# codgodtao/TMDiff

Hardware: AMD Instinct MI355X
Metric: UNet denoise-steps/sec (8-ch 64x64, batch 32) (higher is better)
Workload: dtype f32; 1 GPU; BASELINE configs[1]: batch-32 8-ch 64x64 tiles, DDPM p_sample steps of the T=1000 cosine schedule, channel_multiplier [32,64,128,256], full UNet forward (both branches) + fused DDPM update per step; batch_per_gpu=32, parallelism=batch-parallel x1, weights=key-hashed random init, text_embedding=fixed synthetic 768-d

## Files before the change

include/tmdiff_hip.h:

```cpp
#ifndef TMDIFF_HIP_H
#define TMDIFF_HIP_H

#include <stddef.h>
#include <stdint.h>

#ifdef __cplusplus
extern "C" {
#endif

#define TMDIFF_ABI_VERSION 6

#define TMDIFF_OK 0
#define TMDIFF_E_INVALID (-1)
#define TMDIFF_E_UNSUPPORTED (-2)
#define TMDIFF_E_LAUNCH (-3)

typedef void* tmdiff_stream_t;

int tmdiff_version(void);
const char* tmdiff_last_error_string(void);

typedef struct tmdiff_conv3d_desc {
  int32_t B, N, H, W;
  int32_t Cin, Cout;
// ... 140 lines not shown
int tmdiff_conv3d_prologue_bwd_add(const tmdiff_conv3d_desc* d, const float* gp, float* const dx_seg[3],
                                   const float* const add_seg[3], float* d_shift, float* d_scale, void* workspace,
                                   tmdiff_stream_t stream);

int tmdiff_stem_fwd(const float* xin, const float* pan, const float* ms, const float* w, const float* bias, float* y,
                    int32_t B, int32_t Cout, int32_t N, int32_t H, int32_t W, int32_t apply_silu,
                    tmdiff_stream_t stream);
int tmdiff_stem_fwd_scaled(const float* xin, const float* pan, const float* ms, const float* w, const float* bias,
                           const float* out_scale, int32_t out_scale_stride, float* y, int32_t B, int32_t Cout, int32_t N,
                           int32_t H, int32_t W, int32_t apply_silu, tmdiff_stream_t stream);
int tmdiff_stem_fwd_pack_bf16(const float* xin, const float* pan, const float* ms, const float* w, const float* bias,
                              const float* out_scale, int32_t out_scale_stride, void* units, int32_t B, int32_t Cout, int32_t N,
                              int32_t H, int32_t W, int32_t apply_silu, tmdiff_stream_t stream);
int tmdiff_head_fwd(const float* x, const float* w, const float* scale, int32_t scale_stride, float* y, int32_t B,
                    int32_t C, int64_t P, tmdiff_stream_t stream);
int tmdiff_stem_bwd(const float* xin, const float* pan, const float* ms, const float* w, const float* bias,
                    const float* gy, float* dwb, int32_t B, int32_t Cout, int32_t N, int32_t H, int32_t W,
                    tmdiff_stream_t stream);
int tmdiff_stem_bwd_input(const float* xin, const float* pan, const float* ms, const float* w, const float* bias,
                          const float* gy, float* dx, float* dpan, int32_t B, int32_t Cout, int32_t N, int32_t H,
                          int32_t W, tmdiff_stream_t stream);
int tmdiff_head_bwd(const float* x, const float* w, const float* scale, const float* gy, float* dx, float* dws,
                    int32_t B, int32_t C, int64_t P, tmdiff_stream_t stream);

typedef struct tmdiff_plane_prologue {
  const float* shift;
  const float* scale;
  int32_t shift_stride, scale_stride;
  int32_t C, n_per_channel;
  int32_t act;
} tmdiff_plane_prologue;
int tmdiff_haar_dwt2d_pro(const float* x, float* ll, float* lh, float* hl, float* hh, int64_t planes, int32_t H, int32_t W,
                          float ll_scale, float hi_scale, const tmdiff_plane_prologue* ll_prologue, tmdiff_stream_t stream);
int tmdiff_haar_idwt2d_pro(const float* const ll[2], int32_t n_ll, const float* lh, const float* hl, const float* hh,
                           int64_t hi_planes_per_batch, int64_t hi_batch_stride, float* const out[2], int64_t planes,
                           int32_t h, int32_t w, float in_scale, const tmdiff_plane_prologue* out0_prologue,
                           tmdiff_stream_t stream);
int tmdiff_haar_dwt2d_pack_bf16(const float* x, void* ll_units, float* lh, float* hl, float* hh, int32_t B, int32_t C,
                                int32_t N, int32_t H, int32_t W, float ll_scale, float hi_scale,
                                const tmdiff_plane_prologue* ll_prologue, tmdiff_stream_t stream);
int tmdiff_haar_idwt2d_pack_bf16(const float* ll0, const float* ll1, const float* stacked_bands, void* out0_units, float* out1,
                                 int32_t B, int32_t C, int32_t N, int32_t h, int32_t w, float in_scale,
                                 const tmdiff_plane_prologue* out0_prologue, tmdiff_stream_t stream);
int tmdiff_haar_dwt2d(const float* x, float* ll, float* lh, float* hl, float* hh, int64_t planes, int32_t H,
                      int32_t W, float ll_scale, float hi_scale, tmdiff_stream_t stream);
int tmdiff_haar_idwt2d(const float* const ll[2], int32_t n_ll, const float* lh, const float* hl, const float* hh,
                       int64_t hi_planes_per_batch, int64_t hi_batch_stride, float* const out[2], int64_t planes,
                       int32_t h, int32_t w, float in_scale, tmdiff_stream_t stream);

int tmdiff_linear_fwd(const float* x, const float* w, const float* bias, float* y, int32_t B, int32_t I, int32_t O,
                      int32_t act, tmdiff_stream_t stream);
int tmdiff_gamma_embedding(const float* t, const float* freqs, float* emb, int32_t B, int32_t dim,
                           tmdiff_stream_t stream);
int tmdiff_linear_bwd(const float* x, const float* w, const float* bias, const float* gy, float* gu_scratch,
                      float* dx, float* dw, float* db, int32_t B, int32_t I, int32_t O, int32_t act,
                      tmdiff_stream_t stream);

int tmdiff_ddpm_step(const float* x, const float* eps, const float* noise, const float* ms, float* out,
                     float* img_out, int64_t n, float c_recip, float c_recipm1, float coef1, float coef2,
                     float sigma, int32_t clip, tmdiff_stream_t stream);
int tmdiff_axpby(const float* const in[4], const float coef[4], int32_t n_in, float* out, int64_t n,
                 tmdiff_stream_t stream);
int tmdiff_ddpm_step_dev(const float* x, const float* eps, const float* noise, const float* ms, float* out, float* frames,
                         int64_t n, const int32_t* step, const float* coef, int32_t T, int32_t frame_every, int32_t clip,
                         tmdiff_stream_t stream);
int tmdiff_sampler_tick(int32_t* step, float* time_in, int32_t B, int32_t set_to, tmdiff_stream_t stream);
int tmdiff_ddpm_frame_slot(int32_t t, int32_t T, int32_t frame_every);
typedef struct tmdiff_mt_entry {
  float* out;
  const float* a;
  const float* b;
  int64_t n;
} tmdiff_mt_entry;
int32_t tmdiff_multi_axpby_chunk(void);
int tmdiff_multi_axpby(const tmdiff_mt_entry* tensors_dev, const int32_t* chunk_tensor_dev, const int32_t* chunk_index_dev,
                       int32_t n_chunks, float ca, float cb, tmdiff_stream_t stream);
typedef struct tmdiff_adamw_entry {
  float* p;
  const float* g;
  float* m;
  float* v;
  int64_t n;
} tmdiff_adamw_entry;
int tmdiff_multi_adamw(const tmdiff_adamw_entry* tensors_dev, const int32_t* chunk_tensor_dev, const int32_t* chunk_index_dev,
                       int32_t n_chunks, const float* lr_dev, const float* step_dev, float beta1, float beta2, float eps,
                       float weight_decay, tmdiff_stream_t stream);
size_t tmdiff_multi_sqnorm_workspace_bytes(int32_t n_chunks);
int tmdiff_multi_sqnorm_partial(const tmdiff_adamw_entry* tensors_dev, const int32_t* chunk_tensor_dev,
                                const int32_t* chunk_index_dev, int32_t n_chunks, double* partials_dev, tmdiff_stream_t stream);
int tmdiff_multi_sqnorm_finish(const double* partials_dev, int32_t n_partials, float max_norm, float* norm_dev, float* coef_dev,
                               float* ok_dev, tmdiff_stream_t stream);
int tmdiff_multi_adamw_scaled(const tmdiff_adamw_entry* tensors_dev, const int32_t* chunk_tensor_dev,
                              const int32_t* chunk_index_dev, int32_t n_chunks, const float* lr_dev, const float* step_dev,
                              float beta1, float beta2, float eps, float weight_decay, const float* coef_dev, const float* ok_dev,
                              tmdiff_stream_t stream);
int tmdiff_x0_from_model(const float* x, const float* model_out, float* x0, int64_t n, float alpha, float sigma,
                         int32_t model_is_x_start, tmdiff_stream_t stream);
size_t tmdiff_abs_quantile_workspace_bytes(int32_t B, int64_t n_per_sample);
int tmdiff_abs_quantile_clamp(float* x0, int32_t B, int64_t n_per_sample, float q, float max_val, void* workspace,
                              tmdiff_stream_t stream);
int tmdiff_add(const float* a, const float* b, float* out, int64_t n, float sign_b, tmdiff_stream_t stream);
int tmdiff_q_sample(const float* x0, const float* noise, const float* a, float* out, int32_t B, int64_t n_per_sample,
                    tmdiff_stream_t stream);

int32_t tmdiff_tile_plan(int32_t L, int32_t tile, int32_t overlap, int32_t* origins, int32_t capacity);
int tmdiff_tile_supported(int32_t B, int32_t C, int32_t H, int32_t W, int32_t tile, int32_t overlap);
// ... 112 lines not shown
```

tmdiff_amd/Hyper_unet_general.py:

```python
import math

import torch
import torch.nn as nn

from . import ops, routing

PROMPTS = ("QB", "WV3", "GF2", "WV2", "WV4")

def synthetic_text_embeddings(seed=1234):
    out = {}
    for k, name in enumerate(PROMPTS):
        g = torch.Generator(device="cpu").manual_seed(seed + k)
        out[name] = torch.randn(1, 768, generator=g)
    return out


class Swish(nn.Module):

    def forward(self, x):
        raise RuntimeError("Swish is fused into the HIP kernels; it is never called as a module")



_MASK_FN = None
# ... 512 lines not shown
    @staticmethod
    def _tensor_key(t):
        return (t.data_ptr(), t._version, tuple(t.shape), tuple(t.stride()))

    def begin_condition_cache(self, PAN, MS, prompt):
        with torch.no_grad():
            self._cond = self._condition(self._prepare(), PAN, MS, prompt)
        self._cond["key"] = (self._tensor_key(PAN), self._tensor_key(MS), prompt)

    def add_condition_cache(self, PAN, MS, prompt):
        P = self._prepare()
        if self._cond is None:
            raise RuntimeError("add_condition_cache: no open condition cache (call begin_condition_cache first)")
        with torch.no_grad():
            cond = self._condition(P, PAN, MS, prompt)
        cond["key"] = (self._tensor_key(PAN), self._tensor_key(MS), prompt)
        self._cond.setdefault("more", []).append(cond)

    def end_condition_cache(self):
        self._cond = None

    def invalidate_prepared(self):
        self._prep = None
        self._cond = None
        self.__dict__.pop("_train_pack", None)
        self.__dict__.pop("_train_pack_wino", None)
        self.__dict__.pop("_train_pack_bf16", None)

    _DERIVED = ("_train_pack", "_train_pack_wino", "_train_pack_bf16", "_emb_dev", "_freqs_dev", "_side_stream")

    def __getstate__(self):
        state = {k: v for k, v in self.__dict__.items() if k not in self._DERIVED}
        state["_prep"] = state["_cond"] = None
        return state

    def forward(self, x_t, t_input, PAN=None, MS=None, prompt=None):
        if torch.is_grad_enabled() and (any(p.requires_grad for p in self.parameters()) or any(
                torch.is_tensor(t) and t.requires_grad for t in (x_t, PAN, MS))):
            return self.forward_train(x_t, t_input, PAN, MS, prompt)
        with torch.no_grad():
            return self._forward_infer(x_t, t_input, PAN, MS, prompt)

    def _forward_infer(self, x_t, t_input, PAN, MS, prompt):
        P = self._prepare()
        cond = self._cond
        key = (self._tensor_key(PAN), self._tensor_key(MS), prompt)
        if cond is not None and cond.get("key") != key:
            cond = next((c for c in cond.get("more", ()) if c["key"] == key), None)
        if cond is None:
            cond = self._condition(P, PAN, MS, prompt)
        b = x_t.shape[0]
        t = t_input.reshape(-1).to(device=x_t.device, dtype=torch.float32)
        t = (t if t.numel() == b else t.expand(b)).contiguous()
        g = ops.gamma_embedding(t, P["freqs"], self.inter_dim)
        e = ops.linear(g, self.embed[0].weight.detach(), self.embed[0].bias.detach(), act=True)
        temb = ops.linear(e, self.embed[2].weight.detach(), self.embed[2].bias.detach(), act=True)
        S = {"shift": P["shift_bank"].run(temb), "scale": cond["scale"]}

        fuse_c, fuse = self._producer_fuse(P)
        spec = lambda **k: self._spec(P, S, **k) if fuse_c else None
        h, hp = self._stem(P, S, "conv2", "down1.conv20.dense1", xin=x_t.contiguous())
        hs = [h]
        for dn, nxt in (("down1", "down2.conv20"), ("down2", "down3.conv20"), ("down3", "middle1")):
            h, ha, hq, s2d = self._resblock(P, S, dn + ".conv20", [h], flag=False, pre=hp, emit=spec(), want_ll=True, to_conv0=True)
            h, hp, _ = self._down(P, S, dn + ".down", h, flag=False, want_high=False, pre=ha,
                                  emit=spec(shift=nxt + ".dense1"), fuse=fuse, xq=hq, s2d=s2d)
            hs.append(h)
        h, _ = self._resblock(P, S, "middle1", [hs[3]], flag=False, pre=hp)
        for lvl, upn in ((3, "up1"), (2, "up2"), (1, "up3")):
            h, ha = self._resblock(P, S, upn + ".conv20", [h, cond[f"h{lvl}"], hs[lvl]], flag=False, emit=spec())
            h = self._up(P, S, upn + ".up1", h, cond[f"bands{lvl}"], pre=ha, fuse=fuse)
        h, hp = self._resblock(P, S, "final.conv20", [h, cond["h0"], hs[0]], flag=False, emit=spec(shift="final.conv21.dense1"))
        for k in (1, 2, 3):
            h, hp = self._resblock(P, S, f"final.conv2{k}", [h], flag=False, pre=hp,
                                   emit=spec(shift=f"final.conv2{k + 1}.dense1") if k < 3 else None)
        sc = self._spec(P, S, scale="final.dense2")
        return ops.head(h, self.final.conv24.weight.detach().reshape(-1), sc["scale"], sc["scale_stride"])

    def forward_train(self, x_t, t_input, PAN=None, MS=None, prompt=None):
        from . import autograd as A
        dev = x_t.device
        if dev.type != "cuda":
            raise RuntimeError("tmdiff_amd.WavBEST runs on the HIP kernels only: move the module to a GPU (.cuda())")
        b = x_t.shape[0]
        pk = self.__dict__.get("_train_pack")
        if pk is None or pk.convs[0][0].device != dev:
            self.__dict__.pop("_train_pack_bf16", None)
            pk = self.__dict__["_train_pack"] = ops.PackedWeights(
                [(m.weight, m.groups) for m in self.modules()
                 if isinstance(m, nn.Conv3d) and m.in_channels > 1 and m.out_channels > 1])
        ops.PACKED = pk.refresh()
        wk = self.__dict__.get("_train_pack_wino")
        if wk is None:
            wk = self.__dict__["_train_pack_wino"] = ops.WinoPackedWeights(owner=[w for w, _ in pk.convs])
        ops.WINO_PACKED = wk.refresh() if ops.config.wino_multipack else None
        if ops.config.grad_bf16 and "_train_pack_bf16" not in self.__dict__:
            self.__dict__["_train_pack_bf16"] = ops.Bf16DgradWeights(owner=[w for w, _ in pk.convs])
        ops.BF16_DGRAD = self.__dict__["_train_pack_bf16"] if ops.config.grad_bf16 else None
        lin = lambda seq, i, x, act: A.linear(x, seq[i].weight, seq[i].bias, act=act)
        pe = self._prompt_rows(prompt, b, dev)
        pemb = lin(self.embed2, 4, lin(self.embed2, 2, lin(self.embed2, 0, pe, True), True), True)
        t = t_input.reshape(-1).to(device=dev, dtype=torch.float32)
        t = (t if t.numel() == b else t.expand(b)).contiguous()
        fr = self.__dict__.get("_freqs_dev")
        if fr is None or fr.device != dev:
            fr = self.__dict__["_freqs_dev"] = self._freqs_cpu.to(dev)
        g = ops.gamma_embedding(t, fr, self.inter_dim)
        temb = lin(self.embed, 2, lin(self.embed, 0, g, True), True)

        shift_layers, scale_layers = self._projection_layers()
# ... 50 lines not shown
```

tmdiff_amd/_lib.py:

```python
import ctypes as C
import os

_HERE = os.path.dirname(os.path.abspath(__file__))
LIB_PATH = os.environ.get("TMDIFF_HIP_LIB") or os.path.join(_HERE, "libtmdiff_hip.so")

c_float_p = C.POINTER(C.c_float)
vp = C.c_void_p


class Conv3dDesc(C.Structure):
    _fields_ = [
        ("B", C.c_int32), ("N", C.c_int32), ("H", C.c_int32), ("W", C.c_int32),
        ("Cin", C.c_int32), ("Cout", C.c_int32),
        ("groups", C.c_int32), ("ksize", C.c_int32), ("nseg", C.c_int32),
        ("seg_c", C.c_int32 * 3),
        ("seg_x", vp * 3),
        ("w_packed", vp), ("bias", vp), ("bias_scale", C.c_float),
        ("in_shift", vp), ("in_scale", vp), ("in_shift_stride", C.c_int32), ("in_scale_stride", C.c_int32),
        ("in_mask", vp), ("in_act", C.c_int32),
        ("residual", vp), ("out_scale", C.c_float),
        ("y", vp),
        ("y2", vp), ("y2_shift", vp), ("y2_scale", vp), ("y2_shift_stride", C.c_int32), ("y2_scale_stride", C.c_int32),
        ("y2_act", C.c_int32), ("y2_bf16", C.c_int32), ("x_bf16", C.c_int32),
        ("splitk_ws", vp), ("splitk_ws_bytes", C.c_int64),
# ... 27 lines not shown
    "tmdiff_conv3d_wf_workspace_bytes": (C.c_size_t, [C.POINTER(Conv3dDesc)]),
    "tmdiff_conv3d_wf_splitk_workspace_bytes": (C.c_size_t, [C.POINTER(Conv3dDesc)]),
    "tmdiff_conv3d_wf_fwd": (C.c_int, [C.POINTER(Conv3dDesc), vp, vp]),
    "tmdiff_conv3d_wino_fwd": (C.c_int, [C.POINTER(Conv3dDesc), vp, vp]),
    "tmdiff_conv3d_wino_fwd_planes": (C.c_int, [C.POINTER(Conv3dDesc), vp, C.c_int32, vp, C.c_int32, vp]),
    "tmdiff_conv3d_wino_fwd_xp": (C.c_int, [C.POINTER(Conv3dDesc), vp, C.c_int32, vp, vp]),
    "tmdiff_conv3d_wino_fwd_stage": (C.c_int, [C.POINTER(Conv3dDesc), vp, C.c_int32, vp]),
    "tmdiff_conv3d_prologue_fwd": (C.c_int, [C.POINTER(Conv3dDesc), vp, vp]),
    "tmdiff_conv3d_ll_supported": (C.c_int, [C.POINTER(Conv3dDesc)]),
    "tmdiff_conv3d_ll_splitk_workspace_bytes": (C.c_size_t, [C.POINTER(Conv3dDesc)]),
    "tmdiff_conv3d_ll_packed_bytes": (C.c_size_t, [C.c_int32, C.c_int32]),
    "tmdiff_conv3d_ll_pack_weights": (C.c_int, [vp, vp, C.c_int32, C.c_int32, C.c_float, vp]),
    "tmdiff_conv3d_ll_fwd": (C.c_int, [C.POINTER(Conv3dDesc), C.c_float, vp]),
    "tmdiff_conv3d_packed_bf16_bytes": (C.c_size_t, [C.c_int32, C.c_int32, C.c_int32, C.c_int32]),
    "tmdiff_conv3d_pack_weights_bf16": (C.c_int, [vp, vp, C.c_int32, C.c_int32, C.c_int32, C.c_int32, vp]),
    "tmdiff_conv3d_bf16_workspace_bytes": (C.c_size_t, [C.POINTER(Conv3dDesc)]),
    "tmdiff_conv3d_fwd_bf16": (C.c_int, [C.POINTER(Conv3dDesc), vp, vp]),
    "tmdiff_conv3d_wgrad_workspace_bytes": (C.c_size_t, [C.POINTER(Conv3dDesc)]),
    "tmdiff_conv3d_wgrad": (C.c_int, [C.POINTER(Conv3dDesc), vp, vp, vp, vp]),
    "tmdiff_conv3d_wgrad_bias": (C.c_int, [C.POINTER(Conv3dDesc), vp, vp, vp, vp, vp]),
    "tmdiff_conv3d_wf_plan": (C.c_int32, [C.c_int32] * 8 + [C.POINTER(C.c_int64)]),
    "tmdiff_conv3d_wfll_supported": (C.c_int, [C.POINTER(Conv3dDesc)]),
    "tmdiff_conv3d_wfll_packed_bytes": (C.c_size_t, [C.c_int32, C.c_int32]),
    "tmdiff_conv3d_wfll_pack_weights": (C.c_int, [vp, vp, C.c_int32, C.c_int32, C.c_float, vp]),
    "tmdiff_conv3d_wfll_splitk_workspace_bytes": (C.c_size_t, [C.POINTER(Conv3dDesc)]),
    "tmdiff_conv3d_wfll_fwd": (C.c_int, [C.POINTER(Conv3dDesc), C.c_float, vp]),
    "tmdiff_conv3d_wgrad_wino_supported": (C.c_int, [C.POINTER(Conv3dDesc)]),
    "tmdiff_conv3d_wgrad_wino_workspace_bytes": (C.c_size_t, [C.POINTER(Conv3dDesc)]),
    "tmdiff_conv3d_wgrad_wino": (C.c_int, [C.POINTER(Conv3dDesc), vp, vp, vp, vp]),
    "tmdiff_conv3d_wgrad_wino_bias": (C.c_int, [C.POINTER(Conv3dDesc), vp, vp, vp, vp, vp]),
    "tmdiff_conv3d_pack_weights_bf16_dgrad": (C.c_int, [vp, vp, C.c_int32, C.c_int32, C.c_int32, C.c_int32, vp]),
    "tmdiff_conv3d_wgrad_bf16_supported": (C.c_int, [C.POINTER(Conv3dDesc)]),
    "tmdiff_conv3d_wgrad_bf16_workspace_bytes": (C.c_size_t, [C.POINTER(Conv3dDesc)]),
    "tmdiff_conv3d_wgrad_bf16_slots": (C.c_int32, [C.POINTER(Conv3dDesc)]),
    "tmdiff_conv3d_wgrad_bf16": (C.c_int, [C.POINTER(Conv3dDesc), vp, vp, vp, vp, vp]),
    "tmdiff_channel_sum": (C.c_int, [vp, vp, C.c_int32, C.c_int32, C.c_int64, C.c_float, vp]),
    "tmdiff_conv3d_prologue_bwd": (C.c_int, [C.POINTER(Conv3dDesc), vp, vp * 3, C.c_int32 * 3, vp, vp, vp]),
    "tmdiff_conv3d_prologue_bwd_workspace_bytes": (C.c_size_t, [C.POINTER(Conv3dDesc)]),
    "tmdiff_conv3d_prologue_bwd_ws": (C.c_int, [C.POINTER(Conv3dDesc), vp, vp * 3, C.c_int32 * 3, vp, vp, vp, vp]),
    "tmdiff_conv3d_prologue_bwd_add": (C.c_int, [C.POINTER(Conv3dDesc), vp, vp * 3, vp * 3, vp, vp, vp, vp]),
    "tmdiff_stem_bwd": (C.c_int, [vp, vp, vp, vp, vp, vp, vp, C.c_int32, C.c_int32, C.c_int32, C.c_int32, C.c_int32, vp]),
    "tmdiff_stem_bwd_input": (C.c_int, [vp, vp, vp, vp, vp, vp, vp, vp, C.c_int32, C.c_int32, C.c_int32, C.c_int32, C.c_int32,
                                        vp]),
    "tmdiff_head_bwd": (C.c_int, [vp, vp, vp, vp, vp, vp, C.c_int32, C.c_int32, C.c_int64, vp]),
    "tmdiff_linear_bwd": (C.c_int, [vp, vp, vp, vp, vp, vp, vp, vp, C.c_int32, C.c_int32, C.c_int32, C.c_int32, vp]),
    "tmdiff_stem_fwd": (C.c_int, [vp, vp, vp, vp, vp, vp, C.c_int32, C.c_int32, C.c_int32, C.c_int32, C.c_int32,
                                  C.c_int32, vp]),
    "tmdiff_head_fwd": (C.c_int, [vp, vp, vp, C.c_int32, vp, C.c_int32, C.c_int32, C.c_int64, vp]),
    "tmdiff_haar_dwt2d": (C.c_int, [vp, vp, vp, vp, vp, C.c_int64, C.c_int32, C.c_int32, C.c_float, C.c_float, vp]),
    "tmdiff_haar_idwt2d": (C.c_int, [vp * 2, C.c_int32, vp, vp, vp, C.c_int64, C.c_int64, vp * 2, C.c_int64,
                                     C.c_int32, C.c_int32, C.c_float, vp]),
    "tmdiff_linear_fwd": (C.c_int, [vp, vp, vp, vp, C.c_int32, C.c_int32, C.c_int32, C.c_int32, vp]),
    "tmdiff_gamma_embedding": (C.c_int, [vp, vp, vp, C.c_int32, C.c_int32, vp]),
    "tmdiff_ddpm_step": (C.c_int, [vp, vp, vp, vp, vp, vp, C.c_int64, C.c_float, C.c_float, C.c_float, C.c_float,
                                   C.c_float, C.c_int32, vp]),
    "tmdiff_ddpm_step_dev": (C.c_int, [vp, vp, vp, vp, vp, vp, C.c_int64, vp, vp, C.c_int32, C.c_int32, C.c_int32, vp]),
    "tmdiff_sampler_tick": (C.c_int, [vp, vp, C.c_int32, C.c_int32, vp]),
    "tmdiff_ddpm_frame_slot": (C.c_int, [C.c_int32, C.c_int32, C.c_int32]),
    "tmdiff_axpby": (C.c_int, [vp * 4, C.c_float * 4, C.c_int32, vp, C.c_int64, vp]),
    "tmdiff_multi_axpby_chunk": (C.c_int32, []),
    "tmdiff_multi_axpby": (C.c_int, [vp, vp, vp, C.c_int32, C.c_float, C.c_float, vp]),
    "tmdiff_multi_adamw": (C.c_int, [vp, vp, vp, C.c_int32, vp, vp, C.c_float, C.c_float, C.c_float, C.c_float, vp]),
    "tmdiff_multi_sqnorm_workspace_bytes": (C.c_size_t, [C.c_int32]),
    "tmdiff_multi_sqnorm_partial": (C.c_int, [vp, vp, vp, C.c_int32, vp, vp]),
    "tmdiff_multi_sqnorm_finish": (C.c_int, [vp, C.c_int32, C.c_float, vp, vp, vp, vp]),
    "tmdiff_multi_adamw_scaled": (C.c_int, [vp, vp, vp, C.c_int32, vp, vp, C.c_float, C.c_float, C.c_float, C.c_float, vp, vp,
                                            vp]),
    "tmdiff_x0_from_model": (C.c_int, [vp, vp, vp, C.c_int64, C.c_float, C.c_float, C.c_int32, vp]),
    "tmdiff_abs_quantile_workspace_bytes": (C.c_size_t, [C.c_int32, C.c_int64]),
    "tmdiff_abs_quantile_clamp": (C.c_int, [vp, C.c_int32, C.c_int64, C.c_float, C.c_float, vp, vp]),
    "tmdiff_add": (C.c_int, [vp, vp, vp, C.c_int64, C.c_float, vp]),
    "tmdiff_attn_fwd": (C.c_int, [vp, vp, vp, vp, vp, C.c_int32, C.c_int32, C.c_int32, C.c_int32, C.c_int32,
                                  C.c_int64 * 3, C.c_int64 * 3, C.c_int64 * 3, C.c_int64 * 3, C.c_float, vp]),
    "tmdiff_attn_ctx_queries_per_workgroup": (C.c_int32, [C.c_int32] * 5),
    "tmdiff_attn_fwd_lse": (C.c_int, [vp, vp, vp, vp, vp, C.c_int32, C.c_int32, C.c_int32, C.c_int32, C.c_int32,
                                      C.c_int64 * 3, C.c_int64 * 3, C.c_int64 * 3, C.c_int64 * 3, C.c_float, vp, vp]),
    "tmdiff_attn_bwd_supported": (C.c_int, [C.c_int32] * 5),
    "tmdiff_attn_bwd_workspace_bytes": (C.c_size_t, [C.c_int32] * 5),
    "tmdiff_attn_bwd": (C.c_int, [vp] * 11 + [C.c_int32] * 5 + [C.c_int64 * 3] * 4 + [C.c_float, vp]),
    "tmdiff_gemm_nt": (C.c_int, [vp, vp, vp, vp, vp, C.c_int64, C.c_int32, C.c_int32, vp]),
    "tmdiff_group_norm": (C.c_int, [vp, vp, vp, vp, C.c_int32, C.c_int32, C.c_int64, C.c_int32, C.c_float, vp]),
    "tmdiff_layer_norm": (C.c_int, [vp, vp, vp, vp, C.c_int64, C.c_int32, C.c_float, vp]),
    "tmdiff_geglu": (C.c_int, [vp, vp, C.c_int64, C.c_int32, C.c_int32, vp]),
    "tmdiff_layer_norm_stats": (C.c_int, [vp] * 6 + [C.c_int64, C.c_int32, C.c_float, vp]),
    "tmdiff_group_norm_stats": (C.c_int, [vp] * 6 + [C.c_int32, C.c_int32, C.c_int64, C.c_int32, C.c_float, vp]),
    "tmdiff_layer_norm_bwd_supported": (C.c_int, [C.c_int64, C.c_int32]),
    "tmdiff_layer_norm_bwd_workspace_bytes": (C.c_size_t, [C.c_int64, C.c_int32]),
    "tmdiff_layer_norm_bwd": (C.c_int, [vp] * 9 + [C.c_int64, C.c_int32, vp]),
    "tmdiff_group_norm_bwd_supported": (C.c_int, [C.c_int32, C.c_int32, C.c_int64, C.c_int32]),
    "tmdiff_group_norm_bwd_workspace_bytes": (C.c_size_t, [C.c_int32, C.c_int32, C.c_int64, C.c_int32]),
    "tmdiff_group_norm_bwd": (C.c_int, [vp] * 9 + [C.c_int32, C.c_int32, C.c_int64, C.c_int32, vp]),
    "tmdiff_geglu_bwd": (C.c_int, [vp, vp, vp, C.c_int64, C.c_int32, C.c_int32, vp]),
    "tmdiff_q_sample": (C.c_int, [vp, vp, vp, vp, C.c_int32, C.c_int64, vp]),
    "tmdiff_conv3d_k3_fwd": (C.c_int, [C.POINTER(Conv3dDesc), vp]),
    "tmdiff_conv3d_k3_dgrad": (C.c_int, [C.POINTER(Conv3dDesc), vp]),
    "tmdiff_conv3d_k3_wgrad": (C.c_int, [C.POINTER(Conv3dDesc), vp, vp, vp, vp]),
    "tmdiff_conv3d_k1_fwd": (C.c_int, [C.POINTER(Conv3dDesc), vp]),
    "tmdiff_conv3d_k1_dgrad": (C.c_int, [C.POINTER(Conv3dDesc), vp]),
    "tmdiff_conv3d_k1_wgrad": (C.c_int, [C.POINTER(Conv3dDesc), vp, vp, vp, vp]),
    "tmdiff_haar_dwt2d_fwd": (C.c_int, [vp, vp, vp, vp, vp, C.c_int64, C.c_int32, C.c_int32, C.c_float, C.c_float, vp]),
    "tmdiff_haar_dwt2d_bwd": (C.c_int, [vp, vp, vp, vp, vp, C.c_int64, C.c_int32, C.c_int32, C.c_float, C.c_float, vp]),
    "tmdiff_haar_idwt2d_fwd": (C.c_int, [vp, vp, vp, vp, vp, C.c_int64, C.c_int32, C.c_int32, C.c_float, vp]),
    "tmdiff_haar_idwt2d_bwd": (C.c_int, [vp, vp, vp, vp, vp, C.c_int64, C.c_int32, C.c_int32, C.c_float, vp]),
    "tmdiff_dpm_axpby2": (C.c_int, [vp, C.c_float, vp, C.c_float, vp, C.c_int64, vp]),
    "tmdiff_dpm_axpby3": (C.c_int, [vp, C.c_float, vp, C.c_float, vp, C.c_float, vp, C.c_int64, vp]),
    "tmdiff_dpm_axpby4": (C.c_int, [vp, C.c_float, vp, C.c_float, vp, C.c_float, vp, C.c_float, vp, C.c_int64, vp]),
# ... 75 lines not shown
```

tmdiff_amd/csrc/pointwise.hip:

```cpp
#include "common.h"

namespace {

template <int V>
__global__ void __launch_bounds__(256) stem_kernel(const float* __restrict__ xin, const float* __restrict__ pan,
                                                   const float* __restrict__ ms, const float* __restrict__ w,
                                                   const float* __restrict__ bias, float* __restrict__ y, int Cout,
                                                   long P, long HW, int act, const float* __restrict__ oscale,
                                                   int oscale_stride) {
  const long pv = (blockIdx.x * 256L + threadIdx.x) * V;
  const int b = blockIdx.y;
  if (pv >= P) return;
  float x[V];
  if (ms) {
    const float* m = ms + b * P + pv;
    const float* q = pan + b * HW + pv % HW;
    if constexpr (V == 4) {
      const float4 mv = *reinterpret_cast<const float4*>(m), qv = *reinterpret_cast<const float4*>(q);
      x[0] = qv.x - mv.x, x[1] = qv.y - mv.y, x[2] = qv.z - mv.z, x[3] = qv.w - mv.w;
    } else {
      x[0] = q[0] - m[0];
    }
  } else {
    if constexpr (V == 4) {
// ... 92 lines not shown
                                                     const float* __restrict__ bias, float* __restrict__ y, int B,
                                                     int I, int O, int act) {
  const int lane = threadIdx.x & 63;
  const int o = blockIdx.x * 4 + (threadIdx.x >> 6);
  if (o >= O) return;
  float wr[16];
#pragma unroll
  for (int k = 0; k < 16; ++k) {
    const int i = lane + 64 * k;
    wr[k] = i < I ? w[(long)o * I + i] : 0.f;
  }
  const float bo = bias ? bias[o] : 0.f;
  for (int b0 = 0; b0 < B; b0 += 4) {
    float s[4] = {0.f, 0.f, 0.f, 0.f};
#pragma unroll
    for (int k = 0; k < 16; ++k) {
      const int i = lane + 64 * k;
      if (i < I) {
#pragma unroll
        for (int r = 0; r < 4; ++r)
          if (b0 + r < B) s[r] = fmaf(wr[k], x[(long)(b0 + r) * I + i], s[r]);
      }
    }
#pragma unroll
    for (int off = 32; off > 0; off >>= 1)
#pragma unroll
      for (int r = 0; r < 4; ++r) s[r] += __shfl_xor(s[r], off, 64);
    if (lane == 0) {
#pragma unroll
      for (int r = 0; r < 4; ++r)
        if (b0 + r < B) {
          float v = s[r] + bo;
          if (act) v = tmdiff::silu_f(v);
          y[(long)(b0 + r) * O + o] = v;
        }
    }
  }
}

__global__ void __launch_bounds__(256) gamma_kernel(const float* __restrict__ t, const float* __restrict__ freqs,
                                                    float* __restrict__ emb, int B, int dim) {
  const int half = dim / 2;
  const int i = blockIdx.x * 256 + threadIdx.x;
  if (i >= B * dim) return;
  const int b = i / dim, k = i % dim;
  float v = 0.f;
  if (k < half)
    v = cosf(__fmul_rn(t[b], freqs[k]));
  else if (k < 2 * half)
    v = sinf(__fmul_rn(t[b], freqs[k - half]));
  emb[i] = v;
}

}

extern "C" int tmdiff_stem_fwd(const float* xin, const float* pan, const float* ms, const float* w, const float* bias,
                               float* y, int32_t B, int32_t Cout, int32_t N, int32_t H, int32_t W, int32_t apply_silu,
                               tmdiff_stream_t stream) {
  return tmdiff_stem_fwd_scaled(xin, pan, ms, w, bias, nullptr, 0, y, B, Cout, N, H, W, apply_silu, stream);
}

extern "C" int tmdiff_stem_fwd_scaled(const float* xin, const float* pan, const float* ms, const float* w, const float* bias,
                                      const float* out_scale, int32_t out_scale_stride, float* y, int32_t B, int32_t Cout,
                                      int32_t N, int32_t H, int32_t W, int32_t apply_silu, tmdiff_stream_t stream) {
  using namespace tmdiff;
  const int oss = bank_stride(out_scale_stride, Cout);
  TMDIFF_REQUIRE(B >= 0 && Cout > 0 && N > 0 && H > 0 && W > 0 && B <= 65535, "stem_fwd: bad extents");
  if (B == 0) return TMDIFF_OK;
  TMDIFF_REQUIRE(w && y, "stem_fwd: NULL weights/output");
  TMDIFF_REQUIRE((ms && pan) || (!ms && xin), "stem_fwd: give either (pan, ms) or xin");
  const long HW = (long)H * W, P = HW * N;
  const bool vec = HW % 4 == 0 && aligned16(xin) && aligned16(pan) && aligned16(ms) && aligned16(y);
  if (vec) {
    dim3 grid((unsigned)((P / 4 + 255) / 256), B);
    stem_kernel<4><<<grid, 256, 0, as_stream(stream)>>>(xin, pan, ms, w, bias, y, Cout, P, HW, apply_silu, out_scale, oss);
  } else {
    dim3 grid((unsigned)((P + 255) / 256), B);
    stem_kernel<1><<<grid, 256, 0, as_stream(stream)>>>(xin, pan, ms, w, bias, y, Cout, P, HW, apply_silu, out_scale, oss);
  }
  return check_launch("stem_fwd");
}

extern "C" int tmdiff_stem_fwd_pack_bf16(const float* xin, const float* pan, const float* ms, const float* w,
                                         const float* bias, const float* out_scale, int32_t out_scale_stride, void* units,
                                         int32_t B, int32_t Cout, int32_t N, int32_t H, int32_t W, int32_t apply_silu,
                                         tmdiff_stream_t stream) {
  using namespace tmdiff;
  TMDIFF_REQUIRE(B >= 0 && Cout > 0 && Cout % 8 == 0 && N > 0 && H > 0 && W > 0 && B <= 65535, "stem_fwd_pack_bf16: bad extents");
  if (B == 0) return TMDIFF_OK;
  TMDIFF_REQUIRE(w && units && aligned16(units), "stem_fwd_pack_bf16: NULL / unaligned weights / output");
  TMDIFF_REQUIRE((ms && pan) || (!ms && xin), "stem_fwd_pack_bf16: give either (pan, ms) or xin");
  const int oss = bank_stride(out_scale_stride, Cout);
  const long HW = (long)H * W, P = HW * N;
  stem_pack_bf16_kernel<<<dim3((unsigned)((P + 255) / 256), B), 256, 0, as_stream(stream)>>>(
      xin, pan, ms, w, bias, static_cast<uint4*>(units), Cout, P, HW, apply_silu, out_scale, oss);
  return check_launch("stem_fwd_pack_bf16");
}

extern "C" int tmdiff_head_fwd(const float* x, const float* w, const float* scale, int32_t scale_stride, float* y,
                               int32_t B, int32_t C, int64_t P, tmdiff_stream_t stream) {
  using namespace tmdiff;
  TMDIFF_REQUIRE(B >= 0 && C > 0 && C <= 4096 && P > 0 && B <= 65535, "head_fwd: bad extents B=%d C=%d", B, C);
  if (B == 0) return TMDIFF_OK;
  TMDIFF_REQUIRE(x && w && y, "head_fwd: NULL pointer");
  const int ss = bank_stride(scale_stride, C);
  const bool vec = P % 4 == 0 && aligned16(x) && aligned16(y);
  if (vec) {
    dim3 grid((unsigned)((P / 4 + 255) / 256), B);
    head_kernel<4><<<grid, 256, C * sizeof(float), as_stream(stream)>>>(x, w, scale, ss, y, C, P);
  } else {
    dim3 grid((unsigned)((P + 255) / 256), B);
    head_kernel<1><<<grid, 256, C * sizeof(float), as_stream(stream)>>>(x, w, scale, ss, y, C, P);
  }
  return check_launch("head_fwd");
}

extern "C" int tmdiff_linear_fwd(const float* x, const float* w, const float* bias, float* y, int32_t B, int32_t I,
                                 int32_t O, int32_t act, tmdiff_stream_t stream) {
  using namespace tmdiff;
  TMDIFF_REQUIRE(B >= 0 && I > 0 && I <= 1024 && O > 0, "linear_fwd: B=%d I=%d (<=1024) O=%d", B, I, O);
  if (B == 0) return TMDIFF_OK;
  TMDIFF_REQUIRE(x && w && y, "linear_fwd: NULL pointer");
  linear_kernel<<<(O + 3) / 4, 256, 0, as_stream(stream)>>>(x, w, bias, y, B, I, O, act);
  return check_launch("linear_fwd");
}

extern "C" int tmdiff_gamma_embedding(const float* t, const float* freqs, float* emb, int32_t B, int32_t dim,
                                      tmdiff_stream_t stream) {
  using namespace tmdiff;
  TMDIFF_REQUIRE(B >= 0 && dim >= 2, "gamma_embedding: B=%d dim=%d", B, dim);
  if (B == 0) return TMDIFF_OK;
  TMDIFF_REQUIRE(t && freqs && emb, "gamma_embedding: NULL pointer");
  gamma_kernel<<<(B * dim + 255) / 256, 256, 0, as_stream(stream)>>>(t, freqs, emb, B, dim);
  return check_launch("gamma_embedding");
}
```

tmdiff_amd/ops.py:

```python
import ctypes as C
import math
import os

import numpy as np
import torch

from . import _lib, routing
from ._lib import Conv3dDesc, check, lib



class KernelConfig:

    _FLAG = lambda default: (lambda v: (v != "0") if default else (v == "1"))
    _FIELDS = {
        "winograd": ("TMDIFF_WINOGRAD", _FLAG(True), True), "wf": ("TMDIFF_WF", _FLAG(True), True),
        "wf_pair": ("TMDIFF_WF_PAIR", _FLAG(True), True), "wf_splitk": ("TMDIFF_WF_SPLITK", _FLAG(True), True),
        "wf_min_fill": ("TMDIFF_WF_MIN_FILL", float, 0.7), "wino_min_blocks": ("TMDIFF_WINO_MIN_BLOCKS", int, 256),
        "ll_compose": ("TMDIFF_LL_COMPOSE", _FLAG(True), True), "wfll": ("TMDIFF_WFLL", _FLAG(True), True),
        "train_ll_wino": ("TMDIFF_TRAIN_LL_WINO", _FLAG(True), True),
        "conv2_after_ll": ("TMDIFF_CONV2_AFTER_LL", _FLAG(True), True),
        "epilogue_fuse": ("TMDIFF_EPILOGUE_FUSE", _FLAG(True), True), "producer_fuse": ("TMDIFF_PRODUCER_FUSE", _FLAG(True), True),
        "fp32_staged": ("TMDIFF_FP32_STAGED", str, "auto"), "bf16_pack": ("TMDIFF_BF16_PACK", str, "auto"),
        "wgrad_wino": ("TMDIFF_WGRAD_WINO", _FLAG(True), True), "wgrad_wino_bias": ("TMDIFF_WGRAD_WINO_BIAS", _FLAG(True), True),
        "wgrad_bias": ("TMDIFF_WGRAD_BIAS", _FLAG(False), False), "wino_multipack": ("TMDIFF_WINO_MULTIPACK", _FLAG(True), True),
        "fuse_res_conv": ("TMDIFF_FUSE_RES_CONV", _FLAG(True), True), "emit_ll": ("TMDIFF_EMIT_LL", _FLAG(True), True),
        "emit_dwt": ("TMDIFF_EMIT_DWT", _FLAG(True), True), "side_xp": ("TMDIFF_SIDE_XP", _FLAG(True), True),
        "train_fused_resblock": ("TMDIFF_TRAIN_FUSED_RESBLOCK", _FLAG(True), True),
        "train_graph": ("TMDIFF_TRAIN_GRAPH", _FLAG(False), False),
        "train_two_streams": ("TMDIFF_TRAIN_STREAMS", _FLAG(True), True),
        "sample_graph": ("TMDIFF_SAMPLE_GRAPH", _FLAG(False), False),
        "grad_bf16": ("TMDIFF_GRAD_BF16", _FLAG(False), False),
    }

    def __init__(self, env=None):
        env = os.environ if env is None else env
        for name, (var, parse, default) in self._FIELDS.items():
            object.__setattr__(self, name, parse(env[var]) if var in env else default)

    def __setattr__(self, name, value):
        if name not in self._FIELDS:
            raise AttributeError(f"ops.config has no switch {name!r}")
        object.__setattr__(self, name, value)

    def key(self):
        return tuple(getattr(self, n) for n in self._FIELDS)

    def as_dict(self):
        return {n: getattr(self, n) for n in self._FIELDS}

    def override(self, **values):
        import contextlib

        @contextlib.contextmanager
        def ctx():
            old = {k: getattr(self, k) for k in values}
            try:
                for k, v in values.items():
                    setattr(self, k, v)
                yield self
            finally:
                for k, v in old.items():
                    setattr(self, k, v)
        return ctx()


config = KernelConfig()


_raw_stream = getattr(torch._C, "_cuda_getCurrentRawStream", None)


def stream_ptr():
    if _raw_stream is not None:
        return _raw_stream(torch.cuda.current_device())
    return torch.cuda.current_stream().cuda_stream


def _chk(t, name):
    if t is None:
# ... 669 lines not shown


def haar_idwt2d(lls, lh, hl, hh, in_scale=1.0, outs=None, stacked_bands=None, out0_prologue=None, pack_bf16=False):
    ll0 = lls[0]
    h, w = ll0.shape[-2:]
    planes = ll0.numel() // (h * w)
    if pack_bf16:
        if len(lls) != 2 or stacked_bands is None:
            raise ValueError("haar_idwt2d(pack_bf16=True) takes two low bands and stacked high bands")
        b, c, n = ll0.shape[:3]
        units = torch.empty(b, c // 8, n * 4 * h * w, 8, device=ll0.device, dtype=torch.int16)
        out1 = torch.empty(b, c, n, 2 * h, 2 * w, device=ll0.device, dtype=torch.float32)
        pro = _plane_prologue(out0_prologue, c, n) if out0_prologue is not None else None
        check(lib.tmdiff_haar_idwt2d_pack_bf16(_chk(ll0, "ll0"), _chk(lls[1], "ll1"), _chk(stacked_bands, "bands"),
                                               units.data_ptr(), out1.data_ptr(), b, c, n, h, w, in_scale, pro, stream_ptr()),
              "haar_idwt2d_pack_bf16")
        return [units, out1]
    if outs is None:
        outs = [torch.empty((*ll0.shape[:-2], 2 * h, 2 * w), device=ll0.device, dtype=torch.float32) for _ in lls]
    llp = (C.c_void_p * 2)(*[_chk(t, "ll") for t in lls], *([None] * (2 - len(lls))))
    outp = (C.c_void_p * 2)(*[_chk(t, "out") for t in outs], *([None] * (2 - len(outs))))
    if stacked_bands is not None:
        b = stacked_bands.shape[0]
        ppb = planes // b
        if stacked_bands.numel() != 3 * planes * h * w:
            raise ValueError("haar_idwt2d: stacked bands must be [B, 3C, N, h, w]")
        base = _chk(stacked_bands, "bands")
        step = 4 * ppb * h * w
        hp = (base, base + step, base + 2 * step, ppb, 3 * ppb * h * w)
    else:
        hp = (_chk(lh, "lh"), _chk(hl, "hl"), _chk(hh, "hh"), 0, 0)
    pro = _plane_prologue(out0_prologue, ll0.shape[1], ll0.shape[2]) if out0_prologue is not None else None
    check(lib.tmdiff_haar_idwt2d_pro(llp, len(lls), *hp, outp, planes, h, w, in_scale, pro, stream_ptr()), "haar_idwt2d")
    return outs


def linear(x, w, bias=None, act=False, out=None):
    b, i = x.shape
    o = w.shape[0]
    y = out if out is not None else torch.empty(b, o, device=x.device, dtype=torch.float32)
    check(lib.tmdiff_linear_fwd(_chk(x, "x"), _chk(w, "w"), _chk(bias, "bias"), _chk(y, "y"), b, i, o,
                                1 if act else 0, stream_ptr()), "linear_fwd")
    return y


def gamma_embedding(t, freqs, dim, out=None):
    b = t.shape[0]
    y = out if out is not None else torch.empty(b, dim, device=t.device, dtype=torch.float32)
    check(lib.tmdiff_gamma_embedding(_chk(t, "t"), _chk(freqs, "freqs"), _chk(y, "emb"), b, dim, stream_ptr()),
          "gamma_embedding")
    return y


def ddpm_step(x, eps, noise, c_recip, c_recipm1, coef1, coef2, sigma, clip=True, ms=None, out=None, img_out=None):
    y = out if out is not None else torch.empty_like(x)
    check(lib.tmdiff_ddpm_step(_chk(x, "x"), _chk(eps, "eps"), _chk(noise, "noise"), _chk(ms, "ms"), _chk(y, "out"),
                               _chk(img_out, "img_out"), x.numel(), c_recip, c_recipm1, coef1, coef2, sigma,
                               1 if clip else 0, stream_ptr()), "ddpm_step")
    return y


def ddpm_step_dev(x, eps, noise, step, coef, ms=None, out=None, frames=None, frame_every=1, clip=True):
    y = out if out is not None else torch.empty_like(x)
    if step.dtype != torch.int32 or not step.is_cuda or coef.dim() != 2 or coef.shape[1] != 5:
        raise ValueError("ddpm_step_dev: step must be an int32 device word and coef a [T, 5] table")
    check(lib.tmdiff_ddpm_step_dev(_chk(x, "x"), _chk(eps, "eps"), _chk(noise, "noise"), _chk(ms, "ms"), _chk(y, "out"),
                                   _chk(frames, "frames"), x.numel(), step.data_ptr(), _chk(coef, "coef"), coef.shape[0],
                                   frame_every, 1 if clip else 0, stream_ptr()), "ddpm_step_dev")
    return y


def sampler_tick(step, time_in, set_to=-1):
    if step.dtype != torch.int32 or not step.is_cuda:
        raise ValueError("sampler_tick: step must be an int32 device word")
    check(lib.tmdiff_sampler_tick(step.data_ptr(), _chk(time_in, "time_in"), 0 if time_in is None else time_in.numel(),
                                  int(set_to), stream_ptr()), "sampler_tick")


def axpby(tensors, coefs, out=None):
    n_in = len(tensors)
    y = out if out is not None else torch.empty_like(tensors[0])
    ptrs = (C.c_void_p * 4)(*[_chk(t, "in") for t in tensors], *([None] * (4 - n_in)))
    cf = (C.c_float * 4)(*[float(c) for c in coefs], *([0.0] * (4 - n_in)))
    check(lib.tmdiff_axpby(ptrs, cf, n_in, _chk(y, "out"), y.numel(), stream_ptr()), "axpby")
    return y


def chunk_tables(rows, sizes, device, pinned):
    chunk = lib.tmdiff_multi_axpby_chunk()
    ct, ci = [], []
    for k, n in enumerate(sizes):
        nck = (n + chunk - 1) // chunk
        ct += [k] * nck
        ci += list(range(nck))
    host = [torch.tensor([v for row in rows for v in row], dtype=torch.int64), torch.tensor(ct, dtype=torch.int32),
            torch.tensor(ci, dtype=torch.int32)]
    if pinned:
        host = [h.pin_memory() for h in host]
    devt = [h.to(device, non_blocking=pinned) for h in host]
    return devt[0], devt[1], devt[2], len(ct), host if pinned else None


class MultiAxpby:

    def __init__(self, triples):
        triples = [(o, a, b) for o, a, b in triples if o.numel() > 0]
# ... 651 lines not shown
```

Before: 45.33 batch32-steps/s.

## Fuse time-embedding MLP chain and shift bank into one kernel

```diff
diff --git a/include/tmdiff_hip.h b/include/tmdiff_hip.h
--- a/include/tmdiff_hip.h
+++ b/include/tmdiff_hip.h
@@ -216,6 +216,9 @@
                       int32_t act, tmdiff_stream_t stream);
 int tmdiff_gamma_embedding(const float* t, const float* freqs, float* emb, int32_t B, int32_t dim,
                            tmdiff_stream_t stream);
+int tmdiff_embed_chain_fwd(const float* t, const float* freqs, const float* w0, const float* b0, const float* w2,
+                           const float* b2, const float* wb, const float* bb, float* temb, float* shifts, int32_t B,
+                           int32_t dim, int32_t E, int32_t O, tmdiff_stream_t stream);
 int tmdiff_linear_bwd(const float* x, const float* w, const float* bias, const float* gy, float* gu_scratch,
                       float* dx, float* dw, float* db, int32_t B, int32_t I, int32_t O, int32_t act,
                       tmdiff_stream_t stream);
diff --git a/tmdiff_amd/Hyper_unet_general.py b/tmdiff_amd/Hyper_unet_general.py
--- a/tmdiff_amd/Hyper_unet_general.py
+++ b/tmdiff_amd/Hyper_unet_general.py
@@ -588,10 +588,14 @@
         b = x_t.shape[0]
         t = t_input.reshape(-1).to(device=x_t.device, dtype=torch.float32)
         t = (t if t.numel() == b else t.expand(b)).contiguous()
-        g = ops.gamma_embedding(t, P["freqs"], self.inter_dim)
-        e = ops.linear(g, self.embed[0].weight.detach(), self.embed[0].bias.detach(), act=True)
-        temb = ops.linear(e, self.embed[2].weight.detach(), self.embed[2].bias.detach(), act=True)
-        S = {"shift": P["shift_bank"].run(temb), "scale": cond["scale"]}
+        emb = [p.detach() for m in (self.embed[0], self.embed[2]) for p in (m.weight, m.bias)]
+        if ops.config.embed_fused and b <= 65535:
+            _, shifts = ops.embed_chain(t, P["freqs"], *emb, P["shift_bank"].weight, P["shift_bank"].bias)
+        else:
+            g = ops.gamma_embedding(t, P["freqs"], self.inter_dim)
+            temb = ops.linear(ops.linear(g, emb[0], emb[1], act=True), emb[2], emb[3], act=True)
+            shifts = P["shift_bank"].run(temb)
+        S = {"shift": shifts, "scale": cond["scale"]}
 
         fuse_c, fuse = self._producer_fuse(P)
         spec = lambda **k: self._spec(P, S, **k) if fuse_c else None
diff --git a/tmdiff_amd/_lib.py b/tmdiff_amd/_lib.py
--- a/tmdiff_amd/_lib.py
+++ b/tmdiff_amd/_lib.py
@@ -103,6 +103,7 @@
                                      C.c_int32, C.c_int32, C.c_float, vp]),
     "tmdiff_linear_fwd": (C.c_int, [vp, vp, vp, vp, C.c_int32, C.c_int32, C.c_int32, C.c_int32, vp]),
     "tmdiff_gamma_embedding": (C.c_int, [vp, vp, vp, C.c_int32, C.c_int32, vp]),
+    "tmdiff_embed_chain_fwd": (C.c_int, [vp] * 10 + [C.c_int32, C.c_int32, C.c_int32, C.c_int32, vp]),
     "tmdiff_ddpm_step": (C.c_int, [vp, vp, vp, vp, vp, vp, C.c_int64, C.c_float, C.c_float, C.c_float, C.c_float,
                                    C.c_float, C.c_int32, vp]),
     "tmdiff_ddpm_step_dev": (C.c_int, [vp, vp, vp, vp, vp, vp, C.c_int64, vp, vp, C.c_int32, C.c_int32, C.c_int32, vp]),
diff --git a/tmdiff_amd/csrc/pointwise.hip b/tmdiff_amd/csrc/pointwise.hip
--- a/tmdiff_amd/csrc/pointwise.hip
+++ b/tmdiff_amd/csrc/pointwise.hip
@@ -168,6 +168,95 @@
   emb[i] = v;
 }
 
+template <int NK>
+__device__ __forceinline__ void dense_rows(const float* __restrict__ w, const float* __restrict__ bias, const float* xs, int I,
+                                           int o_begin, int o_end, int act, float* ys, float* yg) {
+  constexpr int R = 8;
+  const int lane = threadIdx.x & 63, wv = threadIdx.x >> 6;
+  float xr[NK];
+  int ic[NK];
+#pragma unroll
+  for (int k = 0; k < NK; ++k) {
+    const int i = lane + 64 * k;
+    ic[k] = i < I ? i : I - 1;
+    xr[k] = xs[ic[k]];
+  }
+  for (int o0 = o_begin + R * wv; o0 < o_end; o0 += 4 * R) {
+    float wr[R][NK], s[R];
+    const int ob = min(o0 + (lane & (R - 1)), o_end - 1);
+    const float bl = bias ? bias[ob] : 0.f;
+#pragma unroll
+    for (int r = 0; r < R; ++r) {
+      const float* row = w + (long)min(o0 + r, o_end - 1) * I;
+#pragma unroll
+      for (int k = 0; k < NK; ++k) wr[r][k] = row[ic[k]];
+    }
+#pragma unroll
+    for (int r = 0; r < R; ++r) {
+      s[r] = 0.f;
+#pragma unroll
+      for (int k = 0; k < NK; ++k) {
+        const float t = fmaf(wr[r][k], xr[k], s[r]);
+        s[r] = lane + 64 * k < I ? t : s[r];
+      }
+    }
+#pragma unroll
+    for (int off = 32; off > 0; off >>= 1)
+#pragma unroll
+      for (int r = 0; r < R; ++r) s[r] += __shfl_xor(s[r], off, 64);
+    float mine = s[0];
+#pragma unroll
+    for (int r = 1; r < R; ++r) mine = lane == r ? s[r] : mine;
+    if (lane < R && o0 + lane < o_end) {
+      float v = mine + bl;
+      if (act) v = tmdiff::silu_f(v);
+      if (ys) ys[o0 + lane] = v;
+      if (yg) yg[o0 + lane] = v;
+    }
+  }
+}
+
+__device__ __forceinline__ void dense_rows_any(const float* __restrict__ w, const float* __restrict__ bias, const float* xs, int I,
+                                               int o_begin, int o_end, int act, float* ys, float* yg) {
+  if (I <= 64) dense_rows<1>(w, bias, xs, I, o_begin, o_end, act, ys, yg);
+  else if (I <= 128) dense_rows<2>(w, bias, xs, I, o_begin, o_end, act, ys, yg);
+  else if (I <= 256) dense_rows<4>(w, bias, xs, I, o_begin, o_end, act, ys, yg);
+  else if (I <= 512) dense_rows<8>(w, bias, xs, I, o_begin, o_end, act, ys, yg);
+  else dense_rows<16>(w, bias, xs, I, o_begin, o_end, act, ys, yg);
+}
+
+__global__ void __launch_bounds__(256) embed_chain_kernel(const float* __restrict__ t, const float* __restrict__ freqs,
+                                                          const float* __restrict__ w0, const float* __restrict__ b0,
+                                                          const float* __restrict__ w2, const float* __restrict__ b2,
+                                                          const float* __restrict__ wb, const float* __restrict__ bb,
+                                                          float* __restrict__ temb, float* __restrict__ shifts, int dim,
+                                                          int E, int O, int o_per_wg) {
+  extern __shared__ float lds[];
+  float* g = lds;
+  float* e = g + dim;
+  float* te = e + E;
+  const int b = blockIdx.y, half = dim / 2;
+  const float tb = t[b];
+  for (int k = threadIdx.x; k < dim; k += 256) {
+    float v = 0.f;
+    if (k < half)
+      v = cosf(__fmul_rn(tb, freqs[k]));
+    else if (k < 2 * half)
+      v = sinf(__fmul_rn(tb, freqs[k - half]));
+    g[k] = v;
+  }
+  __syncthreads();
+  dense_rows_any(w0, b0, g, dim, 0, E, 1, e, nullptr);
+  __syncthreads();
+  const int ob = blockIdx.x * o_per_wg;
+#pragma unroll 1
+  for (int bank = 0; bank < 2; ++bank) {
+    dense_rows_any(bank ? wb : w2, bank ? bb : b2, bank ? te : e, E, bank ? ob : 0, bank ? min(O, ob + o_per_wg) : E, bank ? 0 : 1,
+                   bank ? nullptr : te, bank ? shifts + (long)b * O : (blockIdx.x == 0 ? temb + (long)b * E : nullptr));
+    __syncthreads();
+  }
+}
+
 }
 
 extern "C" int tmdiff_stem_fwd(const float* xin, const float* pan, const float* ms, const float* w, const float* bias,
@@ -250,3 +339,20 @@
   gamma_kernel<<<(B * dim + 255) / 256, 256, 0, as_stream(stream)>>>(t, freqs, emb, B, dim);
   return check_launch("gamma_embedding");
 }
+
+extern "C" int tmdiff_embed_chain_fwd(const float* t, const float* freqs, const float* w0, const float* b0, const float* w2,
+                                      const float* b2, const float* wb, const float* bb, float* temb, float* shifts, int32_t B,
+                                      int32_t dim, int32_t E, int32_t O, tmdiff_stream_t stream) {
+  using namespace tmdiff;
+  TMDIFF_REQUIRE(B >= 0 && B <= 65535 && dim >= 2 && dim <= 1024 && E > 0 && E <= 1024 && O > 0,
+                 "embed_chain_fwd: B=%d dim=%d (2..1024) E=%d (<=1024) O=%d", B, dim, E, O);
+  if (B == 0) return TMDIFF_OK;
+  TMDIFF_REQUIRE(t && freqs && w0 && w2 && wb && temb && shifts, "embed_chain_fwd: NULL pointer");
+  const int want = (512 + B - 1) / B, most = (O + 31) / 32;
+  const int slices = want < most ? want : most;
+  const int o_per_wg = ((O + slices - 1) / slices + 31) / 32 * 32;
+  const dim3 grid((unsigned)((O + o_per_wg - 1) / o_per_wg), (unsigned)B);
+  embed_chain_kernel<<<grid, 256, (size_t)(dim + 2 * E) * sizeof(float), as_stream(stream)>>>(t, freqs, w0, b0, w2, b2, wb, bb, temb,
+                                                                                           shifts, dim, E, O, o_per_wg);
+  return check_launch("embed_chain_fwd");
+}
diff --git a/tmdiff_amd/ops.py b/tmdiff_amd/ops.py
--- a/tmdiff_amd/ops.py
+++ b/tmdiff_amd/ops.py
@@ -26,6 +26,7 @@
         "wgrad_bias": ("TMDIFF_WGRAD_BIAS", _FLAG(False), False), "wino_multipack": ("TMDIFF_WINO_MULTIPACK", _FLAG(True), True),
         "fuse_res_conv": ("TMDIFF_FUSE_RES_CONV", _FLAG(True), True), "emit_ll": ("TMDIFF_EMIT_LL", _FLAG(True), True),
         "emit_dwt": ("TMDIFF_EMIT_DWT", _FLAG(True), True), "side_xp": ("TMDIFF_SIDE_XP", _FLAG(True), True),
+        "embed_fused": ("TMDIFF_EMBED_FUSED", _FLAG(True), True),
         "train_fused_resblock": ("TMDIFF_TRAIN_FUSED_RESBLOCK", _FLAG(True), True),
         "train_graph": ("TMDIFF_TRAIN_GRAPH", _FLAG(False), False),
         "train_two_streams": ("TMDIFF_TRAIN_STREAMS", _FLAG(True), True),
@@ -801,6 +802,18 @@
     return y
 
 
+def embed_chain(t, freqs, w0, b0, w2, b2, bank_w, bank_b):
+    b, (e, dim), o = t.shape[0], w0.shape, bank_w.shape[0]
+    if w2.shape != (e, e) or bank_w.shape[1] != e or freqs.numel() != dim // 2:
+        raise ValueError(f"embed_chain: w0 {tuple(w0.shape)}, w2 {tuple(w2.shape)}, bank {tuple(bank_w.shape)}, {freqs.numel()} frequencies")
+    temb = torch.empty(b, e, device=t.device, dtype=torch.float32)
+    shifts = torch.empty(b, o, device=t.device, dtype=torch.float32)
+    check(lib.tmdiff_embed_chain_fwd(_chk(t, "t"), _chk(freqs, "freqs"), _chk(w0, "w0"), _chk(b0, "b0"), _chk(w2, "w2"), _chk(b2, "b2"),
+                                     _chk(bank_w, "bank_w"), _chk(bank_b, "bank_b"), temb.data_ptr(), shifts.data_ptr(), b, dim, e, o,
+                                     stream_ptr()), "embed_chain_fwd")
+    return temb, shifts
+
+
 def ddpm_step(x, eps, noise, c_recip, c_recipm1, coef1, coef2, sigma, clip=True, ms=None, out=None, img_out=None):
     y = out if out is not None else torch.empty_like(x)
     check(lib.tmdiff_ddpm_step(_chk(x, "x"), _chk(eps, "eps"), _chk(noise, "noise"), _chk(ms, "ms"), _chk(y, "out"),
```

New measurement: 45.31 batch32-steps/s, median of 3. No clear change (-0.0%).
